# danspeech/danspeech

Hardware: AMD Instinct MI355X
Metric: audio-seconds/sec (RTFx) recognize() on 10 s clips, batch=32 (higher is better)
Workload: dtype f32 (two-term fp16 split operands, 3 MFMA products, fp32 accumulate)

## Files before the change

danspeech_amd/DanSpeechRecognizer.py:

```python
import warnings

import os
import numpy as np

from .deepspeech.decoder import GreedyDecoder, BeamCTCDecoder
from .errors.recognizer_errors import ModelNotInitialized
from .audio.parsers import SpectrogramAudioParser, InferenceSpectrogramAudioParser, DeviceClips, StagedClips
from . import batch_plan


class NoLmInstantiatedWarning(Warning):
    pass


_DECODER_SETTINGS = ("lm", "alpha", "beta", "labels", "beam_width")


class _StreamingSession(object):

    def __init__(self, secondary_model, string_parts, lm_partials=False):
        self.secondary_model = secondary_model
        self.string_parts = string_parts
        self.lm_partials = lm_partials
        self.beam = None
# ... 65 lines not shown
    def close(self):
        self.stream.close()
        self.state.close()


class _UnmergedDeviceClips(object):

    def __init__(self, batches):
        self.batches = batches

    def __len__(self):
        return sum(len(b) for b in self.batches)


class _BatchJob(object):
    __slots__ = ("order", "probs", "sizes", "count", "model", "ticket", "slot", "collected", "recomputed")

    def __init__(self, order, probs, sizes, count, model):
        self.order, self.probs, self.sizes, self.count, self.model = order, probs, sizes, count, model
        self.ticket = None
        self.slot = 0
        self.collected = self.recomputed = False

    def collect_forward(self):
        if not self.collected:
            self.recomputed = self.model.collect()
            self.collected = True
        return self.recomputed


def _words(text, spans, token_probs, frame_s):
    words, k = [], 0
    while k < len(text):
        if text[k] == " ":
            k += 1
            continue
# ... 95 lines not shown
        if stale:
            self.decoder = self._build_decoder()

    def _side_stream(self, name):
        import torch
        key = (name, self._device_index())
        if key not in _SIDE_STREAMS:
            _SIDE_STREAMS[key] = torch.cuda.Stream(device=key[1])
        self._side_streams[key] = _SIDE_STREAMS[key]
        return _SIDE_STREAMS[key]

    def _stage_batch(self, recordings, parser=None):
        order = batch_plan.longest_first([len(r) for r in recordings])
        return order, (parser or self.audio_parser).stage([recordings[i] for i in order])

    def _enqueue_batch(self, recordings, model=None, parser=None, decode_slot=None, staged=None):
        import torch
        model = model or self.model
        if isinstance(recordings, DeviceClips):
            order = getattr(recordings, "order", None)
            order = np.arange(len(recordings)) if order is None else order
            here = torch.cuda.current_stream(self._device_index())
            if isinstance(staged, torch.cuda.Event):
                here.wait_event(staged)
            recordings.pcm.record_stream(here)
            feats, frames = (parser or self.audio_parser).parse_batch(recordings)
        else:
            if staged is not None:
                order, clips = staged
            else:
                order = batch_plan.longest_first([len(r) for r in recordings])
                clips = [recordings[i] for i in order]
            feats, frames = (parser or self.audio_parser).parse_batch(clips)
        probs, sizes = model.enqueue(feats, torch.from_numpy(frames.astype(np.int32)))
        job = _BatchJob(order, probs, sizes, len(recordings), model)
        if decode_slot is not None and hasattr(self.decoder, "decode_enqueue"):
            job.slot = decode_slot
            if getattr(self.decoder, "on_lane", False):
                job.ticket = self.decoder.decode_enqueue(probs, sizes, slot=decode_slot)
            else:
                side = self._side_stream("decode")
                done = torch.cuda.Event()
                done.record(torch.cuda.current_stream(self._device_index()))
                side.wait_event(done)
                probs.record_stream(side)
                with torch.cuda.stream(side):
                    job.ticket = self.decoder.decode_enqueue(probs, sizes, slot=decode_slot)
        return job

    def _finish_batch(self, job, show_all, warn=True):
        import torch
        recomputed = job.collect_forward()
        side = self._side_stream("decode")
        job.probs.record_stream(side)
        decoded = None
        if getattr(job, "ticket", None) is not None:
            decoded, _ = self.decoder.decode_collect(job.ticket)
            if recomputed:
                decoded = None
        if decoded is None:
            with torch.cuda.stream(side):
                if hasattr(self.decoder, "decode_enqueue"):
                    decoded, _ = self.decoder.decode_collect(self.decoder.decode_enqueue(job.probs, job.sizes, slot=job.slot))
                else:
                    decoded, _ = self.decoder.decode(job.probs, job.sizes)
        if warn and show_all and self.lm == "greedy":
            warnings.warn("You are trying to get all beams but no LM has been instantiated.", NoLmInstantiatedWarning)
        if getattr(self, "keep_last_output", False):
# ... 5 lines not shown

    def transcribe_batch(self, recordings, show_all=False, sample_rate=None, resample="polyphase"):
        if len(recordings) == 0:
            return []
        if sample_rate is not None and int(sample_rate) != int(self.audio_parser.sampling_rate) and not isinstance(recordings, DeviceClips):
            order = batch_plan.longest_first([len(r) for r in recordings])
            clips = self.audio_parser.resample_batch([recordings[i] for i in order], int(sample_rate), resample)
            clips.order = order
            return self._finish_batch(self._enqueue_batch(clips), show_all)
        return self._finish_batch(self._enqueue_batch(recordings), show_all)

    pipeline_lanes = 4
    pipeline_merge_clips = 64
    pipeline_balance_tail = True

    def _lanes(self, count):
        import torch
        while len(self._replicas) < count - 1 and hasattr(self.model, "replica"):
            self._replicas.append((self.model.replica(), SpectrogramAudioParser(self.audio_config, device=self._device_index())))
        handles = [self.model] + [r[0] for r in self._replicas[:count - 1]]
        parsers = [self.audio_parser] + [r[1] for r in self._replicas[:count - 1]]
        streams = [torch.cuda.current_stream(self._device_index())] + [self._side_stream("lane %d" % k) for k in range(1, len(handles))]
        return handles, parsers, streams

    def _set_up_lanes(self, count, searching):
        handles, parsers, streams = self._lanes(count)
        for h in handles:
            if hasattr(h, "set_inflight"):
                h.set_inflight(max(2, len(handles)) if len(handles) > 1 else 1)
        for p, st in zip(parsers, streams):
            p.share_copy_stream = searching
            p.upload_on_compute_stream = True
            p.upload_stream = st
        return handles, parsers, streams

    def _tear_down_lanes(self, handles, parsers):
        for h in handles:
            if hasattr(h, "set_inflight"):
                h.set_inflight(1)
            if hasattr(h, "set_ring_windows"):
                h.set_ring_windows(0)
        for p in parsers:
            p.upload_stream = None

    def _lanes_that_pay(self, most, clips):
        return batch_plan.lanes_that_pay(getattr(self.model, "rnn_hidden_size", 0), getattr(self.model, "rnn_type", "gru"), most, clips)

    def transcribe_batches(self, batches, show_all=False, lanes=None, merge_clips=None):
        import collections
# ... 37 lines not shown
            ahead = torch.cuda.Event()
            ahead.record(caller_stream)
            return (live[0] if len(live) == 1 else _UnmergedDeviceClips(live)), ahead
        merged = live[0] if len(live) == 1 else [clip for b in live for clip in b]
        return merged, (self._stage_batch(merged, parser) if hasattr(parser, "stage") else None)

    def _transcribe_forwards(self, batches, show_all=False, lanes=None, merge_clips=None, total=None):
        import torch
        import collections
        auto_lanes = lanes is None
        lanes = self.pipeline_lanes if auto_lanes else max(1, int(lanes))
        merge_clips = self.pipeline_merge_clips if merge_clips is None else int(merge_clips)
        searching = hasattr(self.decoder, "decode_enqueue") and not getattr(self.decoder, "on_lane", False)
        grouper = batch_plan.ForwardGrouper(batches, merge_clips, lanes, total, self.pipeline_balance_tail,
                                            kind=lambda b: b.pcm.dtype if isinstance(b, DeviceClips) else None)
        handles, parsers, streams = self._lanes(1)
        caller_stream, device_index = streams[0], self._device_index()
        pending, turn, count, job, done = collections.deque(), 0, 0, None, None

        def drain(keep):
            nonlocal done
            while len(pending) > keep:
                done = pending.popleft()
                parts, finished = done
                res = self._finish_batch(finished, show_all) if finished is not None else []
                done = finished = None
                for r in batch_plan.split_results([len(b) for b in parts], res):
                    yield r

        def next_forward(parser):
            parts = grouper.next_group()
# ... 3 lines not shown
        if lanes > 1 or merge_clips > 0:
            from concurrent.futures import ThreadPoolExecutor
            helper = ThreadPoolExecutor(max_workers=1)

        def fetch_ahead(parser):
            if helper is None:
                return next_forward(parser)

            def work():
                torch.cuda.set_device(device_index)
                torch.cuda.set_stream(caller_stream)
                return next_forward(parser)
            return helper.submit(work)

        try:
            handles, parsers, streams = self._set_up_lanes(1, searching)
            ahead = fetch_ahead(parsers[0])
            group = ahead.result() if helper is not None else ahead
            if auto_lanes and group is not None:
                lanes = self._lanes_that_pay(lanes, sum(len(b) for b in group[0]))
            handles, parsers, streams = self._set_up_lanes(lanes, searching)
            grouper.lanes = lanes = len(handles)
            depth = lanes + 1 if searching else lanes
            while group is not None:
                parts, merged, staged = group
                if len(merged):
                    for older in pending:
                        if older[1] is not None and older[1].model is handles[turn]:
                            older[1].collect_forward()
                    if lanes > 1 and hasattr(handles[turn], "set_ring_windows"):
                        busy = sum(1 for _p, j in pending if j is not None and not j.collected and not j.model.ready())
                        inflight, ring_windows = batch_plan.chip_forms(busy, grouper.forwards_to_come(len(parts)), lanes)
                        handles[turn].set_inflight(inflight)
                        handles[turn].set_ring_windows(ring_windows)
                    with torch.cuda.stream(streams[turn]):
                        if isinstance(merged, _UnmergedDeviceClips):
                            streams[turn].wait_event(staged)
                            merged = DeviceClips.merge(merged.batches)
                        job = self._enqueue_batch(merged, handles[turn], parsers[turn], decode_slot=count % (depth + 1), staged=staged)
                    turn = (turn + 1) % lanes
                    count += 1
                pending.append((parts, job))
                job = None
                if helper is None:
                    yield from drain(0)
                ahead = fetch_ahead(parsers[turn])
                yield from drain(depth)
                group = ahead.result() if helper is not None else ahead
            yield from drain(0)
        finally:
            if helper is not None:
                helper.shutdown(wait=True)
            for left in [done[1] if done else None, job] + [pj[1] for pj in pending]:
                if isinstance(left, _BatchJob):
# ... 499 lines not shown
```

danspeech_amd/_native.py:

```python
import ctypes as C
import os

import numpy as np

_HERE = os.path.dirname(os.path.abspath(__file__))
LIB_PATH = os.environ.get("DSMI_LIBRARY") or os.path.join(_HERE, "lib", "libdsmi.so")

RNN_TYPES = {"gru": 0, "lstm": 1, "rnn": 2}
WINDOWS = {"hamming": 0, "hann": 1, "blackman": 2, "bartlett": 3}
PCM_DTYPES = {np.dtype(np.int16): 0, np.dtype(np.float32): 1, np.dtype(np.float64): 2}
WAV_WIDTH_DTYPE = {1: 3, 2: 0, 3: 4, 4: 5}
PCM_STEREO = 16
_PCM_BYTES = (2, 4, 8, 1, 3, 4)
PAD_MODES = {"reflect": 0, "constant": 1}
RESAMPLE_METHODS = {"polyphase": 0, "ratecv": 1}
RESAMPLE_STREAM_MAX = 256
ENDPOINT_MAX = 256
STREAM_MANY_MAX = 256
BEAM_STREAM_MANY_MAX = 4096
ALIGN_MAX_TOKENS = 4096
SPOT_MAX_TOKENS = 128
SPOT_MAX_PHRASES = 4096
SPOT_MAX_HITS = 64
SCORE_MAX_TOKENS = 2048
# ... 92 lines not shown
    "dsmi_stream_forward_many": (C.c_int, [_vp, C.c_int, _vp, _vp, _vp, _vp, _vp, C.c_int, _vp, _vp]),
    "dsmi_features_stream_many": (C.c_int, [_vp, _vp, C.c_int, _vp, C.c_int, _vp, _vp, C.c_int, _vp, _vp]),
    "dsmi_segment": (C.c_int, [_vp, _vp, C.c_int, C.c_int64, C.c_int, C.c_double, C.c_int, C.c_int, _vp, _vp, C.c_int,
                               C.POINTER(C.c_int), _vp, _vp]),
    "dsmi_decoder_create": (C.c_int, [C.c_int, C.POINTER(C.c_char_p), C.c_int, C.c_int, C.POINTER(_vp)]),
    "dsmi_decoder_destroy": (None, [_vp]),
    "dsmi_decoder_last_error": (C.c_char_p, [_vp]),
    "dsmi_decoder_set_lm": (C.c_int, [_vp, C.c_char_p, C.c_double, C.c_double]),
    "dsmi_beam": (C.c_int, [_vp, _vp, _vp, C.c_int, C.c_int, C.c_int, C.c_int, C.c_double, _vp, _vp, _vp, _vp, _vp]),
    "dsmi_forward": (C.c_int, [_vp, _vp, _vp, C.c_int, C.c_int, _vp, _vp, _vp]),
    "dsmi_forward_ready": (C.c_int, [_vp]),
    "dsmi_forward_status": (C.c_int, [_vp]),
    "dsmi_recompute_count": (C.c_int, [_vp]),
    "dsmi_model_set_inflight": (C.c_int, [_vp, C.c_int]),
    "dsmi_model_set_ring_windows": (C.c_int, [_vp, C.c_int]),
    "dsmi_pack_pcm_i16": (C.c_int, [_vp, C.c_int64, _vp]),
    "dsmi_upload": (C.c_int, [C.c_int, _vp, _vp, C.c_int64, _vp]),
    "dsmi_conv_stack": (C.c_int, [_vp, _vp, _vp, C.c_int, C.c_int, _vp, _vp]),
    "dsmi_rnn_layer": (C.c_int, [_vp, C.c_int, _vp, _vp, C.c_int, C.c_int, _vp, _vp]),
    "dsmi_head": (C.c_int, [_vp, _vp, _vp, C.c_int, C.c_int, _vp, _vp]),
    "dsmi_greedy": (C.c_int, [_vp, _vp, _vp, C.c_int, C.c_int, _vp, _vp, _vp, _vp]),
    "dsmi_greedy_enqueue": (C.c_int, [_vp, _vp, _vp, C.c_int, C.c_int, _vp]),
    "dsmi_greedy_collect": (C.c_int, [_vp, _vp, _vp, _vp]),
    "dsmi_set_profiling": (C.c_int, [_vp, C.c_int]),
    "dsmi_stage_time_us": (C.c_double, [_vp, C.c_int]),
    "dsmi_kernel_stats": (C.c_int, [_vp, C.c_int, _i64p, _i64p, C.POINTER(C.c_double), C.POINTER(C.c_double), C.POINTER(C.c_double)]),
    "dsmi_reset_kernel_stats": (C.c_int, [_vp]),
    "dsmi_debug_persist_stamps": (C.c_int, [_vp, C.c_int, C.c_int, C.c_int, _vp, C.c_int64]),
    "dsmi_debug_step_stamps": (C.c_int, [_vp, C.c_int, C.c_int, C.c_int, C.c_int, _vp, C.c_int64]),
    "dsmi_debug_last_rnn_plan": (C.c_int, [_vp, C.c_char_p, C.c_int64]),
# ... 66 lines not shown
    try:
        import torch
        touched = touched or torch.cuda.is_initialized()
    except ImportError:
        pass
    if not touched:
        os.environ["GPU_MAX_HW_QUEUES"] = str(n)
    elif not _hw_queue_note[0]:
        _hw_queue_note[0] = True
        import warnings
        warnings.warn("danspeech_amd: the GPU runtime was initialised before the recognizer was made and GPU_MAX_HW_QUEUES is not set: "
                      "the batch pipeline's streams will share four hardware queues (recognize_batches runs up to 1.6x slower). "
                      "Set GPU_MAX_HW_QUEUES=8 in the environment, or create the Recognizer before the first GPU call.", RuntimeWarning)


_handles = [0]


def lib():
    global _lib
    if _lib is None:
        if not os.path.exists(LIB_PATH):
            raise NativeLibraryMissing(
                "%s not found: build it with `make -C danspeech_amd/csrc` (hipcc, gfx950) or "
                "`python -c 'import __graft_entry__ as g; g.build()'`. There is no CPU fallback." % LIB_PATH)
        L = C.CDLL(LIB_PATH)
        for name, (res, args) in _PROTOS.items():
            fn = getattr(L, name)
            fn.restype = res
            fn.argtypes = args
# ... 1032 lines not shown
```

danspeech_amd/csrc/api.hip:

```cpp
#include "common.h"
#include "model.h"
#include "gate.h"

#include <algorithm>
#include <cstring>

using namespace dsmi;

static int check_lens(dsmi_model* m, const int32_t* lens, int B, int T) {
    for (int i = 0; i < B; ++i) {
        if (lens[i] < 1 || lens[i] > T) return fail(m, DSMI_ERR_INVALID, "length outside 1..T");
        if (i && lens[i] > lens[i - 1]) return fail(m, DSMI_ERR_UNSORTED, "`lengths` array must be sorted in decreasing order");
    }
    return DSMI_OK;
}

static int check_batch(dsmi_model* m, const int32_t* lens, int B, int T) {
    if (!m->finalized) return fail(m, DSMI_ERR_NOT_READY, "dsmi_model_finalize has not been called");
    if (!lens || B < 1 || T < 1) return fail(m, DSMI_ERR_INVALID, "bad batch arguments");
    return check_lens(m, lens, B, T);
}

static int run_conv(dsmi_model* m, const float* feat, int B, int T, int To, int ys, hipStream_t s, const float** out) {
    const float* x = feat;
// ... 131 lines not shown
    return ok;
}

static void run_rnn_layer(dsmi_model* m, int l, GemmLaunch gl, int B, int To, int dst, hipStream_t s) {
    double sumlen = 0;
    for (int i = 0; i < B; ++i) sumlen += m->host_out_lens[i];
    const double GH = (double)m->geom.G * m->desc.rnn_hidden_size, Dd = m->geom.D;
    RnnPlanInput in = rnn_plan_input(m, B, m->gemm_mode == 1 && gl.w_sp);
    RnnPlan plan = plan_rnn_layer(in);
    if (plan.x16) {
        gl.w_sp = m->rnn[l].wih16_sp; gl.bias = m->rnn[l].bih16; gl.N = m->geom16.Np; gl.ldc = m->geom16.Np;
    }
    gl.ev = timer_arm(m, gl.mode == GEMM_A_CONV ? KK_GEMM0 : KK_GEMM, true, 2.0 * Dd * GH * gl.K * sumlen,
                      4.0 * ((double)gl.M * gl.K * (gl.a2 ? 2 : 1) + (double)gl.N * gl.K + (double)gl.M * gl.N));
    DenseHold hold(m->device, m->inflight, DENSE_GEMM, s);
    m->last_xp_wgs = launch_gemm(gl, s);
    m->last_xp_rows = gl.M; m->last_xp_cols = gl.ldc;
    hold.leave();
    if (run_rnn_plan(m, plan, l, B, To, dst, sumlen, s)) return;
    if (plan.x16) {
        gl.w_sp = m->rnn[l].wih_sp; gl.bias = m->rnn[l].bih; gl.N = m->geom.Np; gl.ldc = m->geom.Np; gl.ev = EvPair{};
        m->last_xp_wgs = launch_gemm(gl, s);
        m->last_xp_cols = gl.ldc;
        in.have16 = false;
        plan = plan_rnn_layer(in);
        if (run_rnn_plan(m, plan, l, B, To, dst, sumlen, s)) return;
    }
    in.rnn_mode = 0;
    (void)run_rnn_plan(m, plan_rnn_layer(in), l, B, To, dst, sumlen, s);
}

static GemmLaunch xproj_gemm(dsmi_model* m, int l, int B, int To) {
    GemmLaunch gl{};
    const RnnW& r = m->rnn[l];
    gl.w = r.wih; gl.bias = r.bih; gl.c = m->xp;
    gl.w_sp = m->gemm_mode == 1 ? r.wih_sp : nullptr;
    gl.a_sp = m->a_sp; gl.tile_cnt = m->dense_tiles ? m->tile_counters(dsmi_model::kTileCntGemm) : nullptr; gl.n_cus = m->n_cus;
    gl.M = To * B; gl.N = m->geom.Np; gl.K = r.K; gl.ldw = r.ldw; gl.ldc = m->geom.Np;
    gl.B = B; gl.T = To;
    return gl;
}

static int stage_lens(dsmi_model* m, int B, hipStream_t s) {
    if (B > m->stage_cap) {
        HIP_OK(m, hipDeviceSynchronize());
        if (m->lens_stage) (void)hipHostFree(m->lens_stage);
        m->lens_stage = nullptr;
        const int cap = std::max(B, 64);
        HIP_OK(m, hipHostMalloc((void**)&m->lens_stage, sizeof(int32_t) * (size_t)cap * dsmi_model::kStage, hipHostMallocDefault));
        m->stage_cap = cap;
        for (int i = 0; i < dsmi_model::kStage; ++i) {
            if (!m->stage_ev[i]) HIP_OK(m, hipEventCreateWithFlags(&m->stage_ev[i], hipEventDisableTiming));
// ... 285 lines not shown
```

danspeech_amd/csrc/gate.h:

```cpp
#pragma once
#include "common.h"

#include <mutex>

struct PersistGate;

bool persist_process_lock(int device);
int persist_next_lane(int device);

class GateTurn {
public:
    void wait(int device, hipStream_t s, const dsmi::RnnLaunch& L, int n_cus);
    void record();
    void hold(int device);
private:
    PersistGate* g_ = nullptr;
    std::unique_lock<std::mutex> lk_;
    hipStream_t s_ = nullptr;
    dsmi::RnnLaunch l_;
};

enum DenseScope { DENSE_CONV_STACK, DENSE_CONV_LAYER, DENSE_GEMM };
int dense_token_limit();
class DenseHold {
public:
    DenseHold(int device, int inflight, DenseScope scope, hipStream_t s);
    void leave();
private:
    unsigned* sem_ = nullptr;
    hipStream_t s_ = nullptr;
};
```

danspeech_amd/csrc/gate.hip:

```cpp
#include "gate.h"
#include "gate_plan.h"

#include <fcntl.h>
#include <sys/file.h>
#include <unistd.h>

using namespace dsmi;

struct PersistGate { std::mutex mu; hipEvent_t ev[kMaxLanes] = {nullptr, nullptr, nullptr, nullptr}; hipEvent_t ring_ev[kRingSlots] = {nullptr, nullptr, nullptr, nullptr, nullptr};
                     hipEvent_t full_ev = nullptr;
                     unsigned* turn = nullptr;
                     DeviceGateState st;
                     int lock_fd = -1; bool lock_tried = false; int next_lane = 0; };

__global__ void turn_acquire_kernel(unsigned* turn) {
    if (threadIdx.x != 0) return;
    unsigned spins = 0;
    while (atomicCAS(turn, 0u, 1u) != 0u && ++spins < (1u << 20)) __builtin_amdgcn_s_sleep(32);
}
__global__ void turn_release_kernel(unsigned* turn) {
    if (threadIdx.x == 0) __hip_atomic_store(turn, 0u, __ATOMIC_RELEASE, __HIP_MEMORY_SCOPE_AGENT);
}

__global__ void dense_enter_kernel(unsigned* sem, unsigned limit) {
    if (threadIdx.x != 0) return;
    for (unsigned spins = 0; spins < (1u << 18); ++spins) {
        const unsigned c = __hip_atomic_load(sem, __ATOMIC_RELAXED, __HIP_MEMORY_SCOPE_AGENT);
        if (c < limit && atomicCAS(sem, c, c + 1u) == c) return;
        __builtin_amdgcn_s_sleep(8);
    }
    atomicAdd(sem, 1u);
}
__global__ void dense_leave_kernel(unsigned* sem) {
    if (threadIdx.x == 0) atomicSub(sem, 1u);
}
static int dense_tokens() {
    static const int k = [] {
        const char* e = std::getenv("DSMI_DENSE_TOKENS");
        if (e) return std::atoi(e);
        const char* q = std::getenv("GPU_MAX_HW_QUEUES");
        return q && std::atoi(q) >= 8 ? 1 : 0;
    }();
    return k;
}
int dense_token_limit() { return dense_tokens(); }
static int dense_scope() {
    static const int k = [] { const char* e = exp_env("DSMI_DEBUG_DENSE_SCOPE"); return e ? std::atoi(e) : 0; }();
    return k;
}

static PersistGate* persist_gate(int device) {
    static std::mutex mu;
    static std::map<int, PersistGate*> gates;
    std::lock_guard<std::mutex> lk(mu);
    auto it = gates.find(device);
    if (it != gates.end()) return it->second;
    PersistGate* g = new PersistGate();
    for (int i = 0; i < kMaxLanes; ++i)
        if (hipEventCreateWithFlags(&g->ev[i], hipEventDisableTiming) != hipSuccess) g->ev[i] = nullptr;
    for (int i = 0; i < kRingSlots; ++i)
        if (hipEventCreateWithFlags(&g->ring_ev[i], hipEventDisableTiming) != hipSuccess) g->ring_ev[i] = nullptr;
    if (hipEventCreateWithFlags(&g->full_ev, hipEventDisableTiming) != hipSuccess) g->full_ev = nullptr;
    const char* turns = std::getenv("DSMI_PERSIST_TURNS");
    if (!(turns && std::string(turns) == "events") && g->full_ev) {
        int cur = -1;
        (void)hipGetDevice(&cur);
        if (hipSetDevice(device) != hipSuccess || hipMalloc((void**)&g->turn, 2 * sizeof(unsigned)) != hipSuccess ||
            hipMemset(g->turn, 0, 2 * sizeof(unsigned)) != hipSuccess) g->turn = nullptr;
        if (cur >= 0 && cur != device) (void)hipSetDevice(cur);
    }
    gates[device] = g;
    return g;
}

static unsigned* dense_sem(int device) {
    PersistGate* g = persist_gate(device);
    return g->turn ? g->turn + 1 : nullptr;
}

bool persist_process_lock(int device) {
    const char* shared = std::getenv("DSMI_PERSIST_SHARED");
    if (shared && shared[0] == '1') return true;
    PersistGate* g = persist_gate(device);
// ... 34 lines not shown
    const DeviceGateRecord r = gate_plan_record(g_->st, l_, g_->turn != nullptr);
    if (r.release) hipLaunchKernelGGL(turn_release_kernel, dim3(1), dim3(64), 0, s_, g_->turn);
    for (int i = 0; i < kMaxLanes; ++i)
        if ((r.lanes >> i & 1) && g_->ev[i]) (void)hipEventRecord(g_->ev[i], s_);
    for (int i = 0; i < kRingSlots; ++i)
        if ((r.ring >> i & 1) && g_->ring_ev[i]) (void)hipEventRecord(g_->ring_ev[i], s_);
    if (r.full && g_->full_ev) (void)hipEventRecord(g_->full_ev, s_);
    g_->st = r.after;
    lk_.unlock();
}
void GateTurn::hold(int device) {
    if (!g_) g_ = persist_gate(device);
    lk_ = std::unique_lock<std::mutex>(g_->mu);
}

DenseHold::DenseHold(int device, int inflight, DenseScope scope, hipStream_t s) : s_(s) {
    const bool behind_token = scope == DENSE_GEMM || dense_scope() == (scope == DENSE_CONV_STACK ? 0 : 2);
    if (dense_tokens() > 0 && inflight >= 2 && behind_token) sem_ = dense_sem(device);
    if (sem_) hipLaunchKernelGGL(dense_enter_kernel, dim3(1), dim3(64), 0, s_, sem_, (unsigned)dense_tokens());
}
void DenseHold::leave() {
    if (sem_) hipLaunchKernelGGL(dense_leave_kernel, dim3(1), dim3(64), 0, s_, sem_);
}
```

danspeech_amd/csrc/gate_plan.h:

```cpp
#pragma once
#include "rnn_plan.h"

namespace dsmi {

struct DeviceGateState { int ring_cus[kRingSlots] = {0, 0, 0, 0, 0}; };

struct DeviceGateWait {
    unsigned lanes = 0, ring = 0;
    bool full = false;
    bool acquire = false;
};
struct DeviceGateRecord {
    unsigned lanes = 0, ring = 0;
    bool full = false;
    bool release = false;
    DeviceGateState after;
};

inline DeviceGateWait gate_plan_wait(const DeviceGateState& st, const RnnLaunch& L, int n_cus, bool have_turn) {
    DeviceGateWait w;
    const int first = L.slot0, n = L.nslots;
    if (L.gate == GATE_RING) {
        int others = 0;
        for (int i = 0; i < kRingSlots; ++i) {
// ... 23 lines not shown
    if (L.gate == GATE_RING) {
        for (int i = first; i < first + n && i < kRingSlots; ++i) {
            r.ring |= 1u << i;
            r.after.ring_cus[i] = L.cus;
        }
        return r;
    }
    if (n >= kMaxLanes && have_turn) {
        r.release = r.full = true;
        return r;
    }
    for (int i = first; i < first + n && i < kMaxLanes; ++i) r.lanes |= 1u << i;
    return r;
}

}
```

danspeech_amd/csrc/model.h:

```cpp
#pragma once
#include "common.h"

struct HostTensor {
    std::vector<int64_t> shape;
    std::vector<float> data;
};

struct ConvW { float *wp = nullptr, *bias = nullptr, *bn_a = nullptr, *bn_b = nullptr; uint16_t* wp_sp = nullptr; };

struct RnnW {
    float* wih = nullptr;
    uint16_t* wih_sp = nullptr;
    float* bih = nullptr;
    float* whh[2] = {nullptr, nullptr};
    uint16_t* whh_sp[2] = {nullptr, nullptr};
    float* bhh[2] = {nullptr, nullptr};
    uint16_t* wih16_sp = nullptr; float* bih16 = nullptr; uint16_t* whh16_sp[2] = {nullptr, nullptr};
    float* bn_a = nullptr;
    float* bn_b = nullptr;
    int K = 0, ldw = 0;
};

enum KernelKind { KK_STFT = 0, KK_CONV1, KK_CONV2, KK_CONV3, KK_GEMM0, KK_GEMM, KK_STEP, KK_HEAD, KK_GREEDY, KK_BEAM, KK_PERSIST, KK_COUNT };
struct KernelTimer {
    std::vector<hipEvent_t> free_events;
    std::vector<std::pair<hipEvent_t, hipEvent_t>> pending[KK_COUNT];
    double sum_us[KK_COUNT] = {0};
    int64_t samples[KK_COUNT] = {0};
    int64_t launches[KK_COUNT] = {0};
    double flops[KK_COUNT] = {0};
    double bytes[KK_COUNT] = {0};
};

struct dsmi_model {
    dsmi_model_desc desc{};
    int device = 0;
    bool finalized = false;
    std::string err;
    std::map<std::string, HostTensor> tensors;

    int n_fft = 0, n_freq = 0;
    int conv_fi[3] = {0, 0, 0}, conv_fo[3] = {0, 0, 0};
    int I0 = 0, Hs = 0;
    dsmi::RnnGeom geom{};
    dsmi::RnnGeom geom16{};
    bool have16 = false;
    int ring_windows = 0;
// ... 6 lines not shown
    std::vector<void*> owned;

    int cap_B = 0, cap_T = 0;
    std::vector<void*> ws;
    float* conv_buf[2] = {nullptr, nullptr};
    uint16_t* conv_buf_sp[2] = {nullptr, nullptr};
    float* xp = nullptr;
    float* hbuf[2][2] = {{nullptr, nullptr}, {nullptr, nullptr}};
    float* cst[2] = {nullptr, nullptr};
    float* look_buf = nullptr;
    float* hpack = nullptr;
    uint16_t* hpack_sp = nullptr;
    uint16_t* hpack16 = nullptr;
    uint16_t* a_sp = nullptr;
    int last_xp_rows = 0, last_xp_cols = 0, last_xp_wgs = 0;
    bool dense_tiles = false;
    bool conv_tiles = false;
    enum TileCnt { kTileCntGemm = 0, kTileCntConv0 = 1, kTileCntBlocks = 4 };
    unsigned* tile_cnt = nullptr;
    unsigned* tile_counters(int which) const { return tile_cnt + (size_t)which * dsmi::kDenseCntWords; }
    int last_conv_wgs[3] = {0, 0, 0};
    unsigned* pcnt = nullptr;
    unsigned* perr = nullptr;
    struct FwdSlot {
        const float* feat = nullptr; float* probs = nullptr; std::vector<int32_t> lens; int B = 0, T = 0; void* stream = nullptr;
        hipEvent_t done = nullptr;
        unsigned* err_host = nullptr;
    };
    static constexpr int kFwdRing = 4;
    FwdSlot fwd[kFwdRing];
    int fwd_head = 0, fwd_count = 0;
// ... 67 lines not shown
```

danspeech_amd/csrc/model_build.hip:

```cpp
#include "common.h"
#include "model.h"
#include "gate.h"

#include <algorithm>
#include <cmath>
#include <cstring>

using namespace dsmi;

static thread_local std::string g_create_error;

constexpr float kF16Safe = 60000.f;

extern "C" int dsmi_model_create(const dsmi_model_desc* d, int device, dsmi_model** out) {
    if (!d || !out) { g_create_error = "null argument"; return DSMI_ERR_INVALID; }
    if (d->conv_layers == 0) { g_create_error = "0 convolutional layers configuration not supported by DanSpeech"; return DSMI_ERR_CONV; }
    if (d->conv_layers > 3 || d->conv_layers < 0) { g_create_error = "Maximum amount of convolutional layers supported by DanSpeech is 3"; return DSMI_ERR_CONV; }
    if (d->rnn_type < 0 || d->rnn_type > 2 || d->rnn_hidden_size < 1 || d->rnn_layers < 1 || d->n_labels < 1 ||
        d->n_labels > 128 || (!d->bidirectional && d->context < 1)) {
        g_create_error = "invalid model description";
        return DSMI_ERR_INVALID;
    }
    int ndev = 0;
    if (hipGetDeviceCount(&ndev) != hipSuccess || device < 0 || device >= ndev) {
// ... 9 lines not shown
    for (int l = 0; l < d->conv_layers; ++l) {
        const ConvSpec& s = kConvSpecs[l];
        m->conv_fi[l] = f;
        f = (f + 2 * s.pf - s.kf) / s.sf + 1;
        m->conv_fo[l] = f;
    }
    m->I0 = kConvSpecs[d->conv_layers - 1].co * f;
    m->geom = make_rnn_geom(d->rnn_type, d->rnn_hidden_size, d->bidirectional ? 2 : 1);
    m->Hs = m->geom.Kp;
    m->geom16 = make_rnn_geom_u(d->rnn_type, d->rnn_hidden_size, d->bidirectional ? 2 : 1, 16);
    m->have16 = d->rnn_hidden_size % 16 == 0;
    m->rnn.resize(d->rnn_layers);
    {
        hipDeviceProp_t prop;
        m->n_cus = hipGetDeviceProperties(&prop, device) == hipSuccess ? prop.multiProcessorCount : 0;
        static const TileSwitches tiles = tile_switches(std::getenv("DSMI_DENSE_TILES"), std::getenv("DSMI_CONV_TILES"), dense_token_limit() > 0);
        m->dense_tiles = tiles.gemm;
        m->conv_tiles = tiles.convs;
        const char* mode = std::getenv("DSMI_RNN_MODE");
        m->rnn_mode = (mode && std::string(mode) == "steps") ? 0 : 1;
        m->persist_gen = (mode && std::string(mode) == "persist8") ? 1 : 2;
        const char* rk = std::getenv("DSMI_RNN_KERNEL");
        m->rnn_kernel = (rk && std::string(rk) == "duo") ? 1 : ((rk && std::string(rk) == "ring") ? 2 : 0);
        m->ring8 = rk && std::string(rk) == "ring8";
        m->ring4 = rk && std::string(rk) == "ring4";
        const char* dm = std::getenv("DSMI_DENSE_MODE");
        const bool dense_f32 = dm && std::string(dm) == "f32";
        m->gemm_mode = dense_f32 ? 0 : 1;
        m->conv_mode = dense_f32 ? 0 : 1;
        m->conv1_split = !dense_f32;
        if (const char* sl = std::getenv("DSMI_DEBUG_SPIN_LIMIT")) m->spin_limit = (unsigned)std::max(1L, std::atol(sl));
        if (const char* ds = std::getenv("DSMI_DEBUG_DROP_SIGNAL"))
            if (std::sscanf(ds, "%d:%d:%d", &m->drop_layer, &m->drop_wg, &m->drop_step) != 3) m->drop_layer = -1;
// ... 285 lines not shown
```

include/dsmi.h:

```cpp
#ifndef DSMI_H
#define DSMI_H

#include <stddef.h>
#include <stdint.h>

#ifdef __cplusplus
extern "C" {
#endif
#if defined(DSMI_BUILD) && defined(__GNUC__)
#pragma GCC visibility push(default)
#endif

typedef enum {
    DSMI_OK = 0,
    DSMI_ERR_INVALID = -1,
    DSMI_ERR_CONV = -2,
    DSMI_ERR_NOT_READY = -3,
    DSMI_ERR_UNSORTED = -4,
    DSMI_ERR_HIP = -5,
    DSMI_ERR_NOMEM = -6,
    DSMI_ERR_IO = -7,
    DSMI_ERR_CAPACITY = -8,
    DSMI_ERR_TIMEOUT = -9,
    DSMI_ERR_COMM = -10,
// ... 109 lines not shown
int dsmi_stream_forward_many(dsmi_stream* const* streams, int n, const float* const* feat_dev, const int* T,
                             const int* is_first, const int* is_last, float* probs_dev, int T_out_cap, int32_t* T_out,
                             void* stream);

int dsmi_segment(dsmi_frontend* f, const void* pcm_dev, int pcm_dtype, int64_t n_samples, int step,
                 double energy_threshold, int pause_hops, int phrase_hops,
                 int64_t* seg_start_host, int64_t* seg_end_host, int max_segments, int* n_segments,
                 double* energies_host, void* stream);

int dsmi_forward(dsmi_model* m, const float* feat_dev, const int32_t* lens_host, int B, int T,
                 float* probs_dev, int32_t* out_lens_host, void* stream);
int dsmi_forward_status(dsmi_model* m);
int dsmi_forward_ready(dsmi_model* m);
int dsmi_model_set_inflight(dsmi_model* m, int batches);
int dsmi_model_set_ring_windows(dsmi_model* m, int windows);
int dsmi_recompute_count(const dsmi_model* m);

int dsmi_conv_stack(dsmi_model* m, const float* feat_dev, const int32_t* lens_host, int B, int T,
                    float* conv_out_dev, void* stream);
int dsmi_rnn_layer(dsmi_model* m, int layer, const float* x_dev, const int32_t* out_lens_host,
                   int B, int T_out, float* y_dev, void* stream);
int dsmi_head(dsmi_model* m, const float* x_fwd_dev, const float* x_rev_dev, int B, int T_out,
              float* probs_dev, void* stream);

int dsmi_decoder_create(int device, const char* const* labels_utf8, int n_labels, int blank_index,
                        dsmi_decoder** out);
void dsmi_decoder_destroy(dsmi_decoder* d);
const char* dsmi_decoder_last_error(const dsmi_decoder* d);

int dsmi_greedy(dsmi_decoder* d, const float* probs_dev, const int32_t* sizes_host, int B, int T_out,
// ... 127 lines not shown
```

Baseline: 63560.

## Create library-owned lane streams, probe hardware independence, gate dense token on proof

Lane and decode streams are now created by the native library, which picks candidates proven to run concurrently. It checks this with a spin/set probe kernel pair launched on the two streams. The dense-GEMM semaphore token and tile counters are enabled only when enough lanes are proven independent, rather than keyed on GPU_MAX_HW_QUEUES. The aim is to avoid deadlock-prone or serialised gating on streams that share a hardware queue, and to give each lane a truly concurrent queue. The cost is probe synchronisation at setup and a more complex stream-management path. The turn acquire now counts give-ups after the spin limit.

```diff
diff --git a/danspeech_amd/DanSpeechRecognizer.py b/danspeech_amd/DanSpeechRecognizer.py
--- a/danspeech_amd/DanSpeechRecognizer.py
+++ b/danspeech_amd/DanSpeechRecognizer.py
@@ -103,12 +103,13 @@
 
 
 class _BatchJob(object):
-    __slots__ = ("order", "probs", "sizes", "count", "model", "ticket", "slot", "collected", "recomputed")
+    __slots__ = ("order", "probs", "sizes", "count", "model", "ticket", "slot", "collected", "recomputed", "decode_stream")
 
     def __init__(self, order, probs, sizes, count, model):
         self.order, self.probs, self.sizes, self.count, self.model = order, probs, sizes, count, model
         self.ticket = None
         self.slot = 0
+        self.decode_stream = None
         self.collected = self.recomputed = False
 
     def collect_forward(self):
@@ -234,7 +235,7 @@
         order = batch_plan.longest_first([len(r) for r in recordings])
         return order, (parser or self.audio_parser).stage([recordings[i] for i in order])
 
-    def _enqueue_batch(self, recordings, model=None, parser=None, decode_slot=None, staged=None):
+    def _enqueue_batch(self, recordings, model=None, parser=None, decode_slot=None, staged=None, decode_stream=None):
         import torch
         model = model or self.model
         if isinstance(recordings, DeviceClips):
@@ -254,12 +255,13 @@
             feats, frames = (parser or self.audio_parser).parse_batch(clips)
         probs, sizes = model.enqueue(feats, torch.from_numpy(frames.astype(np.int32)))
         job = _BatchJob(order, probs, sizes, len(recordings), model)
+        job.decode_stream = decode_stream
         if decode_slot is not None and hasattr(self.decoder, "decode_enqueue"):
             job.slot = decode_slot
             if getattr(self.decoder, "on_lane", False):
                 job.ticket = self.decoder.decode_enqueue(probs, sizes, slot=decode_slot)
             else:
-                side = self._side_stream("decode")
+                side = decode_stream or self._side_stream("decode")
                 done = torch.cuda.Event()
                 done.record(torch.cuda.current_stream(self._device_index()))
                 side.wait_event(done)
@@ -271,7 +273,7 @@
     def _finish_batch(self, job, show_all, warn=True):
         import torch
         recomputed = job.collect_forward()
-        side = self._side_stream("decode")
+        side = job.decode_stream or self._side_stream("decode")
         job.probs.record_stream(side)
         decoded = None
         if getattr(job, "ticket", None) is not None:
@@ -307,17 +309,37 @@
     pipeline_merge_clips = 64
     pipeline_balance_tail = True
 
-    def _lanes(self, count):
+    def _library_streams(self, count, searching):
+        import torch
+        from . import _native
+        dev = self._device_index()
+        caller = torch.cuda.current_stream(dev)
+        handles, _proven, own = _native.lane_streams(dev, count, searching, caller.cuda_stream)
+        streams = []
+        for h in handles:
+            key = ("library", dev, h)
+            if key not in _SIDE_STREAMS:
+                _SIDE_STREAMS[key] = torch.cuda.ExternalStream(h, device=dev)
+            streams.append(_SIDE_STREAMS[key])
+        if own:
+            streams[0] = caller
+        return streams[:count], (streams[count] if searching else None)
+
+    def _lanes(self, count, searching=False):
         import torch
         while len(self._replicas) < count - 1 and hasattr(self.model, "replica"):
             self._replicas.append((self.model.replica(), SpectrogramAudioParser(self.audio_config, device=self._device_index())))
         handles = [self.model] + [r[0] for r in self._replicas[:count - 1]]
         parsers = [self.audio_parser] + [r[1] for r in self._replicas[:count - 1]]
-        streams = [torch.cuda.current_stream(self._device_index())] + [self._side_stream("lane %d" % k) for k in range(1, len(handles))]
-        return handles, parsers, streams
+        decode_stream = None
+        if len(handles) > 1 and hasattr(self.model, "replica"):
+            streams, decode_stream = self._library_streams(len(handles), searching)
+        else:
+            streams = [torch.cuda.current_stream(self._device_index())]
+        return handles, parsers, streams, decode_stream
 
     def _set_up_lanes(self, count, searching):
-        handles, parsers, streams = self._lanes(count)
+        handles, parsers, streams, decode_stream = self._lanes(count, searching)
         for h in handles:
             if hasattr(h, "set_inflight"):
                 h.set_inflight(max(2, len(handles)) if len(handles) > 1 else 1)
@@ -325,7 +347,7 @@
             p.share_copy_stream = searching
             p.upload_on_compute_stream = True
             p.upload_stream = st
-        return handles, parsers, streams
+        return handles, parsers, streams, decode_stream
 
     def _tear_down_lanes(self, handles, parsers):
         for h in handles:
@@ -393,7 +415,7 @@
         searching = hasattr(self.decoder, "decode_enqueue") and not getattr(self.decoder, "on_lane", False)
         grouper = batch_plan.ForwardGrouper(batches, merge_clips, lanes, total, self.pipeline_balance_tail,
                                             kind=lambda b: b.pcm.dtype if isinstance(b, DeviceClips) else None)
-        handles, parsers, streams = self._lanes(1)
+        handles, parsers, streams, decode_stream = self._lanes(1)
         caller_stream, device_index = streams[0], self._device_index()
         pending, turn, count, job, done = collections.deque(), 0, 0, None, None
 
@@ -427,12 +449,12 @@
             return helper.submit(work)
 
         try:
-            handles, parsers, streams = self._set_up_lanes(1, searching)
+            handles, parsers, streams, decode_stream = self._set_up_lanes(1, searching)
             ahead = fetch_ahead(parsers[0])
             group = ahead.result() if helper is not None else ahead
             if auto_lanes and group is not None:
                 lanes = self._lanes_that_pay(lanes, sum(len(b) for b in group[0]))
-            handles, parsers, streams = self._set_up_lanes(lanes, searching)
+            handles, parsers, streams, decode_stream = self._set_up_lanes(lanes, searching)
             grouper.lanes = lanes = len(handles)
             depth = lanes + 1 if searching else lanes
             while group is not None:
@@ -450,7 +472,8 @@
                         if isinstance(merged, _UnmergedDeviceClips):
                             streams[turn].wait_event(staged)
                             merged = DeviceClips.merge(merged.batches)
-                        job = self._enqueue_batch(merged, handles[turn], parsers[turn], decode_slot=count % (depth + 1), staged=staged)
+                        job = self._enqueue_batch(merged, handles[turn], parsers[turn], decode_slot=count % (depth + 1), staged=staged,
+                                                  decode_stream=decode_stream)
                     turn = (turn + 1) % lanes
                     count += 1
                 pending.append((parts, job))
diff --git a/danspeech_amd/_native.py b/danspeech_amd/_native.py
--- a/danspeech_amd/_native.py
+++ b/danspeech_amd/_native.py
@@ -130,6 +130,10 @@
     "dsmi_recompute_count": (C.c_int, [_vp]),
     "dsmi_model_set_inflight": (C.c_int, [_vp, C.c_int]),
     "dsmi_model_set_ring_windows": (C.c_int, [_vp, C.c_int]),
+    "dsmi_lane_streams": (C.c_int, [C.c_int, C.c_int, C.c_int, _vp, C.POINTER(_vp), C.POINTER(C.c_int), C.POINTER(C.c_int)]),
+    "dsmi_lane_streams_release": (C.c_int, [C.c_int]),
+    "dsmi_streams_independent": (C.c_int, [C.c_int, _vp, _vp]),
+    "dsmi_gate_stats": (C.c_int, [C.c_int, C.POINTER(C.c_int), C.POINTER(C.c_int), _i64p, _i64p]),
     "dsmi_pack_pcm_i16": (C.c_int, [_vp, C.c_int64, _vp]),
     "dsmi_upload": (C.c_int, [C.c_int, _vp, _vp, C.c_int64, _vp]),
     "dsmi_conv_stack": (C.c_int, [_vp, _vp, _vp, C.c_int, C.c_int, _vp, _vp]),
@@ -226,6 +230,32 @@
                       "Set GPU_MAX_HW_QUEUES=8 in the environment, or create the Recognizer before the first GPU call.", RuntimeWarning)
 
 
+def lane_streams(device, lanes, searching, caller_stream):
+    n = int(lanes) + (1 if searching else 0)
+    out = (_vp * n)()
+    proven, own = C.c_int(0), C.c_int(0)
+    _handles[0] += 1
+    rc = lib().dsmi_lane_streams(int(device), int(lanes), 1 if searching else 0, _vp(int(caller_stream or 0)), out, C.byref(proven), C.byref(own))
+    if rc != 0:
+        raise DsmiError(rc, "dsmi_lane_streams(device %d, %d lanes)" % (device, lanes))
+    return [int(h or 0) for h in out], proven.value, bool(own.value)
+
+
+def streams_independent(device, a, b):
+    rc = lib().dsmi_streams_independent(int(device), _vp(int(a or 0)), _vp(int(b or 0)))
+    if rc < 0:
+        raise DsmiError(rc, "dsmi_streams_independent(device %d)" % device)
+    return bool(rc)
+
+
+def gate_stats(device):
+    on, proven, takes, gave = C.c_int(0), C.c_int(0), C.c_int64(0), C.c_int64(0)
+    rc = lib().dsmi_gate_stats(int(device), C.byref(on), C.byref(proven), C.byref(takes), C.byref(gave))
+    if rc != 0:
+        raise DsmiError(rc, "dsmi_gate_stats(device %d)" % device)
+    return {"token_on": bool(on.value), "proven_lanes": proven.value, "takes": takes.value, "give_ups": gave.value}
+
+
 _handles = [0]
 
 
diff --git a/danspeech_amd/csrc/api.hip b/danspeech_amd/csrc/api.hip
--- a/danspeech_amd/csrc/api.hip
+++ b/danspeech_amd/csrc/api.hip
@@ -169,6 +169,7 @@
     gl.ev = timer_arm(m, gl.mode == GEMM_A_CONV ? KK_GEMM0 : KK_GEMM, true, 2.0 * Dd * GH * gl.K * sumlen,
                       4.0 * ((double)gl.M * gl.K * (gl.a2 ? 2 : 1) + (double)gl.N * gl.K + (double)gl.M * gl.N));
     DenseHold hold(m->device, m->inflight, DENSE_GEMM, s);
+    gl.tile_cnt = tile_switches(dense_tiles_text(), conv_tiles_text(), hold.token_on()).gemm ? m->tile_counters(dsmi_model::kTileCntGemm) : nullptr;
     m->last_xp_wgs = launch_gemm(gl, s);
     m->last_xp_rows = gl.M; m->last_xp_cols = gl.ldc;
     hold.leave();
@@ -190,7 +191,7 @@
     const RnnW& r = m->rnn[l];
     gl.w = r.wih; gl.bias = r.bih; gl.c = m->xp;
     gl.w_sp = m->gemm_mode == 1 ? r.wih_sp : nullptr;
-    gl.a_sp = m->a_sp; gl.tile_cnt = m->dense_tiles ? m->tile_counters(dsmi_model::kTileCntGemm) : nullptr; gl.n_cus = m->n_cus;
+    gl.a_sp = m->a_sp; gl.tile_cnt = nullptr; gl.n_cus = m->n_cus;
     gl.M = To * B; gl.N = m->geom.Np; gl.K = r.K; gl.ldw = r.ldw; gl.ldc = m->geom.Np;
     gl.B = B; gl.T = To;
     return gl;
diff --git a/danspeech_amd/csrc/gate.h b/danspeech_amd/csrc/gate.h
--- a/danspeech_amd/csrc/gate.h
+++ b/danspeech_amd/csrc/gate.h
@@ -20,13 +20,16 @@
     dsmi::RnnLaunch l_;
 };
 
+bool streams_independent(int device, hipStream_t a, hipStream_t b);
+
 enum DenseScope { DENSE_CONV_STACK, DENSE_CONV_LAYER, DENSE_GEMM };
-int dense_token_limit();
 class DenseHold {
 public:
     DenseHold(int device, int inflight, DenseScope scope, hipStream_t s);
     void leave();
+    bool token_on() const { return on_; }
 private:
     unsigned* sem_ = nullptr;
     hipStream_t s_ = nullptr;
+    bool on_ = false;
 };
diff --git a/danspeech_amd/csrc/gate.hip b/danspeech_amd/csrc/gate.hip
--- a/danspeech_amd/csrc/gate.hip
+++ b/danspeech_amd/csrc/gate.hip
@@ -6,17 +6,40 @@
 #include <unistd.h>
 
 using namespace dsmi;
+
+struct LaneStreams {
+    std::mutex mu;
+    int device = -1;
+    unsigned* words = nullptr;
+    unsigned* seen_host = nullptr;
+    hipEvent_t zeroed = nullptr;
+    std::map<std::pair<hipStream_t, hipStream_t>, bool> probed;
+    bool made = false;
+    int n_cand = 0;
+    hipStream_t cand[kLaneCandidates] = {};
+    int chosen[kLaneCandidates] = {};
+    int n_chosen = 0;
+    hipStream_t granted[kLaneStreamsMax + 1] = {};
+    int n_granted = 0, n_proven = 0, n_lanes = 0;
+    bool searching = false;
+    hipStream_t caller = nullptr; bool caller_proven = false;
+};
 
 struct PersistGate { std::mutex mu; hipEvent_t ev[kMaxLanes] = {nullptr, nullptr, nullptr, nullptr}; hipEvent_t ring_ev[kRingSlots] = {nullptr, nullptr, nullptr, nullptr, nullptr};
                      hipEvent_t full_ev = nullptr;
                      unsigned* turn = nullptr;
                      DeviceGateState st;
-                     int lock_fd = -1; bool lock_tried = false; int next_lane = 0; };
+                     int lock_fd = -1; bool lock_tried = false; int next_lane = 0;
+                     LaneStreams lanes;
+                     std::atomic<long long> takes{0}; };
 
 __global__ void turn_acquire_kernel(unsigned* turn) {
     if (threadIdx.x != 0) return;
     unsigned spins = 0;
-    while (atomicCAS(turn, 0u, 1u) != 0u && ++spins < (1u << 20)) __builtin_amdgcn_s_sleep(32);
+    while (atomicCAS(turn, 0u, 1u) != 0u) {
+        if (++spins >= (1u << 20)) { atomicAdd(turn + 2, 1u); return; }
+        __builtin_amdgcn_s_sleep(32);
+    }
 }
 __global__ void turn_release_kernel(unsigned* turn) {
     if (threadIdx.x == 0) __hip_atomic_store(turn, 0u, __ATOMIC_RELEASE, __HIP_MEMORY_SCOPE_AGENT);
@@ -30,20 +53,19 @@
         __builtin_amdgcn_s_sleep(8);
     }
     atomicAdd(sem, 1u);
+    atomicAdd(sem + 1, 1u);
 }
 __global__ void dense_leave_kernel(unsigned* sem) {
     if (threadIdx.x == 0) atomicSub(sem, 1u);
 }
-static int dense_tokens() {
-    static const int k = [] {
-        const char* e = std::getenv("DSMI_DENSE_TOKENS");
-        if (e) return std::atoi(e);
-        const char* q = std::getenv("GPU_MAX_HW_QUEUES");
-        return q && std::atoi(q) >= 8 ? 1 : 0;
-    }();
+static const char* dense_tokens_text() {
+    static const char* const e = std::getenv("DSMI_DENSE_TOKENS");
+    return e;
+}
+static bool dense_force() {
+    static const bool k = [] { const char* e = exp_env("DSMI_DEBUG_DENSE_FORCE"); return e && std::atoi(e) != 0; }();
     return k;
 }
-int dense_token_limit() { return dense_tokens(); }
 static int dense_scope() {
     static const int k = [] { const char* e = exp_env("DSMI_DEBUG_DENSE_SCOPE"); return e ? std::atoi(e) : 0; }();
     return k;
@@ -65,8 +87,8 @@
     if (!(turns && std::string(turns) == "events") && g->full_ev) {
         int cur = -1;
         (void)hipGetDevice(&cur);
-        if (hipSetDevice(device) != hipSuccess || hipMalloc((void**)&g->turn, 2 * sizeof(unsigned)) != hipSuccess ||
-            hipMemset(g->turn, 0, 2 * sizeof(unsigned)) != hipSuccess) g->turn = nullptr;
+        if (hipSetDevice(device) != hipSuccess || hipMalloc((void**)&g->turn, 4 * sizeof(unsigned)) != hipSuccess ||
+            hipMemset(g->turn, 0, 4 * sizeof(unsigned)) != hipSuccess) g->turn = nullptr;
         if (cur >= 0 && cur != device) (void)hipSetDevice(cur);
     }
     gates[device] = g;
@@ -131,10 +153,198 @@
     lk_ = std::unique_lock<std::mutex>(g_->mu);
 }
 
+__global__ void probe_spin_kernel(unsigned* w) {
+    if (threadIdx.x != 0) return;
+    const unsigned long long t0 = __builtin_amdgcn_s_memrealtime();
+    unsigned seen = 0;
+    for (unsigned polls = 0; polls < (1u << 14); ++polls) {
+        seen = __hip_atomic_load(w, __ATOMIC_RELAXED, __HIP_MEMORY_SCOPE_AGENT);
+        if (seen || __builtin_amdgcn_s_memrealtime() - t0 > 150000ull) break;
+        __builtin_amdgcn_s_sleep(16);
+    }
+    w[1] = seen ? 1u : 2u;
+}
+__global__ void probe_set_kernel(unsigned* w) {
+    if (threadIdx.x == 0) __hip_atomic_store(w, 1u, __ATOMIC_RELAXED, __HIP_MEMORY_SCOPE_AGENT);
+}
+
+static bool probe_once(LaneStreams& ls, hipStream_t a, hipStream_t b) {
+    if (a == b) return false;
+    if (!ls.words) {
+        if (hipMalloc((void**)&ls.words, 2 * sizeof(unsigned)) != hipSuccess) { ls.words = nullptr; return false; }
+        if (hipHostMalloc((void**)&ls.seen_host, sizeof(unsigned), hipHostMallocDefault) != hipSuccess) ls.seen_host = nullptr;
+        if (hipEventCreateWithFlags(&ls.zeroed, hipEventDisableTiming) != hipSuccess) ls.zeroed = nullptr;
+    }
+    if (!ls.seen_host || !ls.zeroed) return false;
+    *ls.seen_host = 0;
+    bool ok = hipMemsetAsync(ls.words, 0, 2 * sizeof(unsigned), a) == hipSuccess && hipEventRecord(ls.zeroed, a) == hipSuccess &&
+              hipStreamWaitEvent(b, ls.zeroed, 0) == hipSuccess;
+    if (ok) {
+        hipLaunchKernelGGL(probe_spin_kernel, dim3(1), dim3(64), 0, a, ls.words);
+        hipLaunchKernelGGL(probe_set_kernel, dim3(1), dim3(64), 0, b, ls.words);
+        ok = hipMemcpyAsync(ls.seen_host, ls.words + 1, sizeof(unsigned), hipMemcpyDeviceToHost, a) == hipSuccess;
+    }
+    const bool sa = hipStreamSynchronize(a) == hipSuccess, sb = hipStreamSynchronize(b) == hipSuccess;
+    return ok && sa && sb && *ls.seen_host == 1u;
+}
+static bool keeps_its_address(const LaneStreams& ls, hipStream_t s) {
+    if (s == nullptr) return true;
+    for (int i = 0; i < ls.n_cand; ++i) if (ls.cand[i] == s) return true;
+    return false;
+}
+static bool probe_cached(LaneStreams& ls, hipStream_t a, hipStream_t b) {
+    if (a == b) return false;
+    if (!keeps_its_address(ls, a) || !keeps_its_address(ls, b)) return probe_once(ls, a, b);
+    auto it = ls.probed.find({a, b});
+    if (it != ls.probed.end()) return it->second;
+    const bool r = probe_once(ls, a, b);
+    ls.probed[{a, b}] = r;
+    return r;
+}
+
+struct OnDevice {
+    int cur = -1; bool ok;
+    explicit OnDevice(int device) { (void)hipGetDevice(&cur); ok = cur == device || hipSetDevice(device) == hipSuccess; if (cur == device) cur = -1; }
+    ~OnDevice() { if (cur >= 0) (void)hipSetDevice(cur); }
+};
+
+bool streams_independent(int device, hipStream_t a, hipStream_t b) {
+    if (a == b) return false;
+    LaneStreams& ls = persist_gate(device)->lanes;
+    std::lock_guard<std::mutex> lk(ls.mu);
+    OnDevice dev(device);
+    return dev.ok && probe_cached(ls, a, b);
+}
+
+static void make_lane_streams(LaneStreams& ls) {
+    if (ls.made) return;
+    ls.made = true;
+    for (int i = 0; i < kLaneCandidates; ++i) {
+        hipStream_t s = nullptr;
+        if (hipStreamCreateWithFlags(&s, hipStreamNonBlocking) != hipSuccess) break;
+        ls.cand[ls.n_cand++] = s;
+    }
+    const int n = ls.n_cand;
+    unsigned char indep[kLaneCandidates * kLaneCandidates] = {};
+    for (int a = 0; a < n; ++a)
+        for (int b = 0; b < n; ++b) indep[a * n + b] = probe_cached(ls, ls.cand[a], ls.cand[b]) ? 1 : 0;
+    for (int round = 0; round <= n * n; ++round) {
+        ls.n_chosen = select_lane_streams(indep, n, kLaneStreamsMax + 1, ls.chosen);
+        bool held = true;
+        for (int i = 0; i < ls.n_chosen; ++i)
+            for (int k = 0; k < ls.n_chosen; ++k) {
+                const int a = ls.chosen[i], b = ls.chosen[k];
+                if (a == b || probe_once(ls, ls.cand[a], ls.cand[b])) continue;
+                indep[a * n + b] = 0; ls.probed[{ls.cand[a], ls.cand[b]}] = false; held = false;
+            }
+        if (held) return;
+    }
+    ls.n_chosen = 0;
+}
+
+static bool granted_proven(const LaneStreams& ls, hipStream_t s) {
+    if (ls.caller_proven && s == ls.caller) return true;
+    for (int i = ls.caller_proven ? 1 : 0; i < ls.n_proven; ++i) if (ls.granted[i] == s) return true;
+    return false;
+}
+
+static int dense_token_for(int device, int inflight, hipStream_t s) {
+    if (dense_force()) return dense_token_decide(dense_tokens_text(), 0, inflight, false, true);
+    if (dense_tokens_text() && dense_token_decide(dense_tokens_text(), 1 << 20, 2, false) == 0) return 0;
+    LaneStreams& ls = persist_gate(device)->lanes;
+    std::lock_guard<std::mutex> lk(ls.mu);
+    if (!ls.n_granted || !granted_proven(ls, s)) return 0;
+    return dense_token_decide(dense_tokens_text(), ls.n_proven, inflight >= 2 ? std::max(inflight, ls.n_lanes) : inflight, ls.searching);
+}
+
+extern "C" int dsmi_streams_independent(int device, void* a, void* b) {
+    int count = 0;
+    if (a == b) return 0;
+    if (hipGetDeviceCount(&count) != hipSuccess || device < 0 || device >= count) return DSMI_ERR_INVALID;
+    return streams_independent(device, (hipStream_t)a, (hipStream_t)b) ? 1 : 0;
+}
+
+extern "C" int dsmi_lane_streams(int device, int lanes, int searching, void* caller_stream, void** streams, int* proven, int* caller_independent) {
+    int count = 0;
+    if (!streams || lanes < 1 || lanes + (searching ? 1 : 0) > kLaneStreamsMax + 1) return DSMI_ERR_INVALID;
+    if (hipGetDeviceCount(&count) != hipSuccess || device < 0 || device >= count) return DSMI_ERR_INVALID;
+    LaneStreams& ls = persist_gate(device)->lanes;
+    std::lock_guard<std::mutex> lk(ls.mu);
+    OnDevice dev(device);
+    if (!dev.ok) return DSMI_ERR_HIP;
+    ls.device = device;
+    make_lane_streams(ls);
+    const int want = lanes + (searching ? 1 : 0);
+    if (ls.n_cand < want) return DSMI_ERR_HIP;
+    int n = 0;
+    for (; n < want && n < ls.n_chosen; ++n) ls.granted[n] = ls.cand[ls.chosen[n]];
+    const int n_proven = n;
+    for (int c = 0; c < ls.n_cand && n < want; ++c) {
+        bool used = false;
+        for (int k = 0; k < ls.n_chosen; ++k) used = used || ls.chosen[k] == c;
+        if (!used) ls.granted[n++] = ls.cand[c];
+    }
+    ls.n_granted = n; ls.n_proven = n_proven; ls.n_lanes = lanes; ls.searching = searching != 0;
+    const hipStream_t c = (hipStream_t)caller_stream;
+    bool c_ok = n_proven >= 1;
+    for (int i = 1; i < n_proven && c_ok; ++i) c_ok = probe_cached(ls, c, ls.granted[i]) && probe_cached(ls, ls.granted[i], c);
+    for (int i = 0; i < n && c_ok; ++i) c_ok = ls.granted[i] != c;
+    ls.caller = c; ls.caller_proven = c_ok;
+    for (int i = 0; i < n; ++i) streams[i] = (void*)ls.granted[i];
+    if (proven) *proven = n_proven;
+    if (caller_independent) *caller_independent = c_ok ? 1 : 0;
+    return DSMI_OK;
+}
+
+extern "C" int dsmi_lane_streams_release(int device) {
+    int count = 0;
+    if (hipGetDeviceCount(&count) != hipSuccess || device < 0 || device >= count) return DSMI_ERR_INVALID;
+    LaneStreams& ls = persist_gate(device)->lanes;
+    std::lock_guard<std::mutex> lk(ls.mu);
+    OnDevice dev(device);
+    if (!dev.ok) return DSMI_ERR_HIP;
+    for (int i = 0; i < ls.n_cand; ++i) { (void)hipStreamSynchronize(ls.cand[i]); (void)hipStreamDestroy(ls.cand[i]); ls.cand[i] = nullptr; }
+    ls.n_cand = ls.n_chosen = ls.n_granted = ls.n_proven = ls.n_lanes = 0;
+    ls.made = ls.searching = ls.caller_proven = false;
+    ls.caller = nullptr;
+    ls.probed.clear();
+    return DSMI_OK;
+}
+
+extern "C" int dsmi_gate_stats(int device, int* token_on, int* proven_lanes, int64_t* takes, int64_t* give_ups) {
+    int count = 0;
+    if (hipGetDeviceCount(&count) != hipSuccess || device < 0 || device >= count) return DSMI_ERR_INVALID;
+    PersistGate* g = persist_gate(device);
+    {
+        LaneStreams& ls = g->lanes;
+        std::lock_guard<std::mutex> lk(ls.mu);
+        const int lanes_proven = std::min(ls.n_proven, ls.n_lanes);
+        if (proven_lanes) *proven_lanes = lanes_proven;
+        if (token_on) *token_on = g->turn && ls.n_granted &&
+                                  (dense_force() ? dense_token_decide(dense_tokens_text(), 0, std::max(2, ls.n_lanes), false, true)
+                                                 : dense_token_decide(dense_tokens_text(), ls.n_proven, std::max(2, ls.n_lanes), ls.searching)) > 0;
+    }
+    if (takes) *takes = g->takes.load(std::memory_order_relaxed);
+    if (give_ups) {
+        unsigned n = 0;
+        OnDevice dev(device);
+        if (g->turn && (!dev.ok || hipDeviceSynchronize() != hipSuccess || hipMemcpy(&n, g->turn + 2, sizeof(unsigned), hipMemcpyDeviceToHost) != hipSuccess))
+            return DSMI_ERR_HIP;
+        *give_ups = n;
+    }
+    return DSMI_OK;
+}
+
 DenseHold::DenseHold(int device, int inflight, DenseScope scope, hipStream_t s) : s_(s) {
     const bool behind_token = scope == DENSE_GEMM || dense_scope() == (scope == DENSE_CONV_STACK ? 0 : 2);
-    if (dense_tokens() > 0 && inflight >= 2 && behind_token) sem_ = dense_sem(device);
-    if (sem_) hipLaunchKernelGGL(dense_enter_kernel, dim3(1), dim3(64), 0, s_, sem_, (unsigned)dense_tokens());
+    const int limit = inflight >= 2 ? dense_token_for(device, inflight, s) : 0;
+    unsigned* sem = limit > 0 ? dense_sem(device) : nullptr;
+    on_ = sem != nullptr;
+    if (on_ && behind_token) sem_ = sem;
+    if (sem_) {
+        hipLaunchKernelGGL(dense_enter_kernel, dim3(1), dim3(64), 0, s_, sem_, (unsigned)limit);
+        persist_gate(device)->takes.fetch_add(1, std::memory_order_relaxed);
+    }
 }
 void DenseHold::leave() {
     if (sem_) hipLaunchKernelGGL(dense_leave_kernel, dim3(1), dim3(64), 0, s_, sem_);
diff --git a/danspeech_amd/csrc/gate_plan.h b/danspeech_amd/csrc/gate_plan.h
--- a/danspeech_amd/csrc/gate_plan.h
+++ b/danspeech_amd/csrc/gate_plan.h
@@ -61,4 +61,32 @@
     return r;
 }
 
+constexpr int kLaneCandidates = 12;
+constexpr int kLaneStreamsMax = 8;
+
+inline bool lane_pair_proven(const unsigned char* indep, int n, int a, int b) {
+    return a != b && indep[a * n + b] && indep[b * n + a];
 }
+inline int select_lane_streams(const unsigned char* indep, int n, int want, int* chosen) {
+    int count = 0;
+    for (int c = 0; c < n && count < want; ++c) {
+        bool ok = true;
+        for (int k = 0; k < count && ok; ++k) ok = lane_pair_proven(indep, n, c, chosen[k]);
+        if (ok) chosen[count++] = c;
+    }
+    return count;
+}
+
+inline int dense_token_decide(const char* text, int proven, int inflight, bool searching, bool force = false) {
+    int limit = 1;
+    if (text && *text) {
+        limit = 0;
+        for (const char* c = text; *c >= '0' && *c <= '9' && limit < 1000; ++c) limit = limit * 10 + (*c - '0');
+        if (limit <= 0) return 0;
+    }
+    if (inflight < 2) return 0;
+    if (force) return limit;
+    return proven >= inflight + (searching ? 1 : 0) ? limit : 0;
+}
+
+}
diff --git a/danspeech_amd/csrc/model.h b/danspeech_amd/csrc/model.h
--- a/danspeech_amd/csrc/model.h
+++ b/danspeech_amd/csrc/model.h
@@ -31,6 +31,9 @@
     double flops[KK_COUNT] = {0};
     double bytes[KK_COUNT] = {0};
 };
+
+inline const char* dense_tiles_text() { static const char* const e = std::getenv("DSMI_DENSE_TILES"); return e; }
+inline const char* conv_tiles_text() { static const char* const e = std::getenv("DSMI_CONV_TILES"); return e; }
 
 struct dsmi_model {
     dsmi_model_desc desc{};
@@ -67,7 +70,6 @@
     uint16_t* hpack16 = nullptr;
     uint16_t* a_sp = nullptr;
     int last_xp_rows = 0, last_xp_cols = 0, last_xp_wgs = 0;
-    bool dense_tiles = false;
     bool conv_tiles = false;
     enum TileCnt { kTileCntGemm = 0, kTileCntConv0 = 1, kTileCntBlocks = 4 };
     unsigned* tile_cnt = nullptr;
diff --git a/danspeech_amd/csrc/model_build.hip b/danspeech_amd/csrc/model_build.hip
--- a/danspeech_amd/csrc/model_build.hip
+++ b/danspeech_amd/csrc/model_build.hip
@@ -47,9 +47,7 @@
     {
         hipDeviceProp_t prop;
         m->n_cus = hipGetDeviceProperties(&prop, device) == hipSuccess ? prop.multiProcessorCount : 0;
-        static const TileSwitches tiles = tile_switches(std::getenv("DSMI_DENSE_TILES"), std::getenv("DSMI_CONV_TILES"), dense_token_limit() > 0);
-        m->dense_tiles = tiles.gemm;
-        m->conv_tiles = tiles.convs;
+        m->conv_tiles = tile_switches(dense_tiles_text(), conv_tiles_text(), false).convs;
         const char* mode = std::getenv("DSMI_RNN_MODE");
         m->rnn_mode = (mode && std::string(mode) == "steps") ? 0 : 1;
         m->persist_gen = (mode && std::string(mode) == "persist8") ? 1 : 2;
diff --git a/include/dsmi.h b/include/dsmi.h
--- a/include/dsmi.h
+++ b/include/dsmi.h
@@ -147,6 +147,10 @@
 int dsmi_forward_ready(dsmi_model* m);
 int dsmi_model_set_inflight(dsmi_model* m, int batches);
 int dsmi_model_set_ring_windows(dsmi_model* m, int windows);
+int dsmi_lane_streams(int device, int lanes, int searching, void* caller_stream, void** streams, int* proven, int* caller_independent);
+int dsmi_lane_streams_release(int device);
+int dsmi_streams_independent(int device, void* a, void* b);
+int dsmi_gate_stats(int device, int* token_on, int* proven_lanes, int64_t* takes, int64_t* give_ups);
 int dsmi_recompute_count(const dsmi_model* m);
 
 int dsmi_conv_stack(dsmi_model* m, const float* feat_dev, const int32_t* lens_host, int B, int T,
```

Result: no change. 63430 (-0.2%).
